# weikaolun/horovod-distributed-example

Hardware: AMD Instinct MI355X
Metric: images/sec (whole node) + scaling efficiency, ResNet-50 bf16 at 1/2/4/8 MI355X (higher is better)
Workload: dtype bf16; 1 GPU; model=ResNet-50, global_batch=2048, per_gpu_batch=2048, image=224, parallelism=dp1, optimizer=mivod FusedSGD via DistributedOptimizer, compression=none, transport=local, hip_graph=False

## Files before the change

csrc/kernels/mv_stem.hip:

```cpp
#include "mv_mfma.h"
#include "mv_stem.h"

namespace mv {
namespace stem {

constexpr int kH = 224, kW = 224, kC = 4, kOH = 112, kOW = 112, kCO = 64;
constexpr int kPW = 232;
constexpr int kChunks = 32;
#ifndef MV_STEM_ROWS
#define MV_STEM_ROWS 2
#endif
constexpr int kR = MV_STEM_ROWS;
constexpr int kIR = 2 * kR + 5;
constexpr int kPatch = kIR * kPW;
constexpr int kLoads = (kIR * 230 + 255) / 256;

__device__ __forceinline__ u32x2 ld_px(const __bf16* x, int64_t pix, int cin) {
  if (cin == 4) return *reinterpret_cast<const u32x2*>(x + pix * 4);
  const uint16_t* p = reinterpret_cast<const uint16_t*>(x) + pix * 3;
  return u32x2{(uint32_t)p[0] | ((uint32_t)p[1] << 16), (uint32_t)p[2]};
}

__global__ __launch_bounds__(256, 2) void stem_fwd_kernel(const __bf16* __restrict__ x,
                                                       const __bf16* __restrict__ w,
                                                       __bf16* __restrict__ z,
                                                       const float* __restrict__ shift,
                                                       float* __restrict__ partial, int N,
                                                       int cin) {
  __shared__ __attribute__((aligned(16))) __bf16 ws[kCO * kChunks * 8];
  __shared__ __attribute__((aligned(16))) __bf16 ps[kPatch * kC];
  const int tid = threadIdx.x, lane = tid & 63, wv = tid >> 6;
  const int g = lane >> 4, rl = lane & 15;

  for (int q = tid; q < kCO * kChunks; q += 256) {
    const int o = q / kChunks, ch = q % kChunks;
    u32x4 v = {0u, 0u, 0u, 0u};
    if (ch < 28) {
      const int r = ch / 4, pr = ch % 4;
      const __bf16* src = w + ((o * 7 + r) * 7 + 2 * pr) * kC;
      const u32x2 a = *reinterpret_cast<const u32x2*>(src);
      v[0] = a[0];
      v[1] = a[1];
      if (pr < 3) {
        const u32x2 b = *reinterpret_cast<const u32x2*>(src + kC);
        v[2] = b[0];
        v[3] = b[1];
      }
    }
    *reinterpret_cast<u32x4*>(ws + (o * kChunks + (ch ^ (o & 7))) * 8) = v;
  }

  const int64_t rows = (int64_t)N * (kOH / kR);
  u32x2 pre[kLoads];
  auto gload = [&](int64_t row) {
    const int n = (int)(row / (kOH / kR)), oh = (int)(row % (kOH / kR)) * kR;
#pragma unroll
    for (int i = 0; i < kLoads; ++i) {
      const int q = tid + i * 256;
      const int r = q / 230, pc = q % 230;
      const int ih = 2 * oh + r - 3, iw = pc - 3;
      u32x2 v = {0u, 0u};
      if (q < kIR * 230 && ih >= 0 && ih < kH && iw >= 0 && iw < kW)
        v = ld_px(x, ((int64_t)n * kH + ih) * kW + iw, cin);
      pre[i] = v;
    }
  };

  float sh[4], s1[4], s2[4];
#pragma unroll
  for (int j = 0; j < 4; ++j) {
    sh[j] = shift ? shift[16 * wv + 4 * g + j] : 0.f;
    s1[j] = 0.f;
    s2[j] = 0.f;
  }
  int64_t row = blockIdx.x;
  if (row < rows) gload(row);
  for (; row < rows; row += gridDim.x) {
    __syncthreads();
#pragma unroll
    for (int i = 0; i < kLoads; ++i) {
      const int q = tid + i * 256;
      if (q < kIR * 230) {
        const int r = q / 230, pc = q % 230;
        *reinterpret_cast<u32x2*>(ps + (r * kPW + pc) * kC) = pre[i];
      }
    }
    __syncthreads();
    if (row + gridDim.x < rows) gload(row + gridDim.x);
    f32x4v acc[kR][7];
#pragma unroll
    for (int j = 0; j < kR; ++j)
#pragma unroll
      for (int t = 0; t < 7; ++t) acc[j][t] = f32x4v{0.f, 0.f, 0.f, 0.f};
#pragma unroll
    for (int kk = 0; kk < 7; ++kk) {
      const int o = 16 * wv + rl, ch = kk * 4 + g;
      const bf16x8 wf = *reinterpret_cast<const bf16x8*>(ws + (o * kChunks + (ch ^ (o & 7))) * 8);
#pragma unroll
      for (int j = 0; j < kR; ++j)
#pragma unroll
        for (int t = 0; t < 7; ++t) {
          const int p = t * 16 + rl;
          const bf16x8 af = *reinterpret_cast<const bf16x8*>(
              ps + ((2 * j + kk) * kPW + 2 * p + 2 * g) * kC);
          acc[j][t] = mfma(wf, af, acc[j][t]);
        }
    }
#pragma unroll
    for (int j = 0; j < kR; ++j)
#pragma unroll
    for (int t = 0; t < 7; ++t) {
      __bf16* zr = z + (row * kR + j) * (int64_t)kOW * kCO + 16 * wv + 4 * g;
      const int p = t * 16 + rl;
      const uint32_t lo = cvt_pk_bf16_cc(acc[j][t][0], acc[j][t][1]);
      const uint32_t hi = cvt_pk_bf16_cc(acc[j][t][2], acc[j][t][3]);
      *reinterpret_cast<u32x2*>(zr + (int64_t)p * kCO) = u32x2{lo, hi};
      const float v[4] = {__uint_as_float(lo << 16), __uint_as_float(lo & 0xffff0000u),
                          __uint_as_float(hi << 16), __uint_as_float(hi & 0xffff0000u)};
#pragma unroll
      for (int e = 0; e < 4; ++e) {
        const float d = v[e] - sh[e];
        s1[e] += d;
        s2[e] += d * d;
      }
    }
  }
#pragma unroll
  for (int j = 0; j < 4; ++j) {
#pragma unroll
    for (int o = 1; o < 16; o <<= 1) {
      s1[j] += __shfl_xor(s1[j], o, kWave);
      s2[j] += __shfl_xor(s2[j], o, kWave);
    }
  }
  if (rl == 0) {
#pragma unroll
    for (int j = 0; j < 4; ++j) {
      const int c = 16 * wv + 4 * g + j;
      partial[((int64_t)blockIdx.x * 2 + 0) * kCO + c] = s1[j];
      partial[((int64_t)blockIdx.x * 2 + 1) * kCO + c] = s2[j];
    }
  }
}

}
}

int mv_stem_partials(int N) {
  static int per = [] {
    int v = 0;
    if (hipOccupancyMaxActiveBlocksPerMultiprocessor(&v, (const void*)mv::stem::stem_fwd_kernel,
                                                     256, 0) != hipSuccess || v < 1)
      v = 1;
    return v;
  }();
  const int64_t rows = (int64_t)N * (mv::stem::kOH / mv::stem::kR);
  int64_t g = (int64_t)mv::num_cus() * per;
  if (g > rows) g = rows;
  return (int)g;
}

void mv_stem_fwd(const void* x, const void* w, void* z, const float* shift, float* partial, int N,
                 hipStream_t st, int grid, int cin) {
  if (grid <= 0) grid = mv_stem_partials(N);
  hipLaunchKernelGGL(mv::stem::stem_fwd_kernel, dim3(grid), dim3(256), 0, st, (const __bf16*)x,
                     (const __bf16*)w, (__bf16*)z, shift, partial, N, cin);
}

namespace mv {
namespace stem {


__device__ __forceinline__ s16x4 px_tr4(const __bf16* ps, int p0, int r, int s0, int c) {
  int p = p0 + (c >> 2);
  p = p < kOW - 1 ? p : kOW - 1;
  const __bf16* a = ps + (r * kPW + 2 * p + s0) * kC + 4 * (c & 3);
  return lds_tr4(a);
}

constexpr int kPairs = (kOW / 2) * 8;

__device__ __forceinline__ void pool_bn_dz_pair(const MvStemPoolBwd& pb, const float* coef, int n,
                                                int oh, int b, int c, const u32x4 (&zr)[2],
                                                u32x4 (&out)[2]) {
  constexpr int kPH = kOH / 2, kPW2 = kOW / 2;
  float acc[2][8];
#pragma unroll
  for (int k = 0; k < 2; ++k)
#pragma unroll
    for (int e = 0; e < 8; ++e) acc[k][e] = 0.f;
  const int a = oh >> 1, i = oh & 1;
  const int nda = i && a + 1 < kPH ? 2 : 1;
  const bool ok1 = b + 1 < kPW2;
  for (int da = 0; da < nda; ++da) {
    const int kh = i - 2 * da + 1;
    u32x2 iw[2];
    u32x4 dv[2], d2v[2];
#pragma unroll
    for (int db = 0; db < 2; ++db) {
      const int col = db && !ok1 ? b : b + db;
      const int64_t o = (((int64_t)n * kPH + a + da) * kPW2 + col) * kCO + c;
      iw[db] = *reinterpret_cast<const u32x2*>(pb.idx + o);
      dv[db] = *reinterpret_cast<const u32x4*>(reinterpret_cast<const __bf16*>(pb.dy) + o);
      d2v[db] = pb.dy2 ? *reinterpret_cast<const u32x4*>(reinterpret_cast<const __bf16*>(pb.dy2) + o)
                       : u32x4{0u, 0u, 0u, 0u};
    }
#pragma unroll
    for (int db = 0; db < 2; ++db) {
      float d[8];
#pragma unroll
      for (int q = 0; q < 4; ++q) {
        d[2 * q] = __uint_as_float(dv[db][q] << 16);
        d[2 * q + 1] = __uint_as_float(dv[db][q] & 0xffff0000u);
      }
      if (pb.dy2) {
#pragma unroll
        for (int q = 0; q < 4; ++q) {
          d[2 * q] += __uint_as_float(d2v[db][q] << 16);
          d[2 * q + 1] += __uint_as_float(d2v[db][q] & 0xffff0000u);
        }
      }
#pragma unroll
      for (int jj = 0; jj < 2; ++jj) {
        const int kw = jj - 2 * db + 1;
        if (kw < 0) continue;
        const uint32_t pos = db && !ok1 ? 0xffu : (uint32_t)(kh * 3 + kw);
#pragma unroll
        for (int e = 0; e < 8; ++e) {
          const uint32_t wd = e < 4 ? iw[db][0] : iw[db][1];
          if (((wd >> (8 * (e & 3))) & 0xffu) == pos) acc[jj][e] += d[e];
        }
      }
    }
  }
#pragma unroll
  for (int k = 0; k < 2; ++k) {
    float v[8];
#pragma unroll
    for (int q = 0; q < 4; ++q) {
      v[2 * q] = __uint_as_float(zr[k][q] << 16);
      v[2 * q + 1] = __uint_as_float(zr[k][q] & 0xffff0000u);
    }
#pragma unroll
    for (int e = 0; e < 8; ++e) {
      const float* kf = coef + c + e;
      const float d = __builtin_fmaf(v[e], kf[0], kf[64]) > 0.f ? acc[k][e] : 0.f;
      v[e] = __builtin_fmaf(kf[128], d, __builtin_fmaf(kf[192], v[e], kf[256]));
    }
    out[k] = u32x4{cvt_pk_bf16(v[0], v[1]), cvt_pk_bf16(v[2], v[3]), cvt_pk_bf16(v[4], v[5]),
                   cvt_pk_bf16(v[6], v[7])};
  }
}

template <int NT, bool FUSE>
__global__ __launch_bounds__(NT, FUSE ? 4 : 1) void stem_wgrad_kernel(const __bf16* __restrict__ x,
                                                        const __bf16* __restrict__ dz,
                                                        float* __restrict__ partial, int N,
                                                        int cin, MvStemPoolBwd pb) {
  static_assert(!FUSE || NT >= kPairs, "one pixel pair per thread");
  constexpr int kTPW = 14 / (NT / 256);
  __shared__ __attribute__((aligned(16))) __bf16 ps[7 * kPW * kC];
  __shared__ __attribute__((aligned(16))) __bf16 ds[128 * 64];
  __shared__ float coef[FUSE ? 5 * 64 : 1];
  const int tid = threadIdx.x;
  if constexpr (FUSE) {
    for (int q = tid; q < 5 * 64; q += NT) {
      const float* src[5] = {pb.scale, pb.bias, pb.ca, pb.cb, pb.cc};
      coef[q] = src[q / 64][q % 64];
    }
  }
  const int64_t rows = (int64_t)N * kOH;
  f32x4v acc[kTPW];
#pragma unroll
  for (int t = 0; t < kTPW; ++t) acc[t] = f32x4v{0.f, 0.f, 0.f, 0.f};
  for (int q = tid; q < 16 * 8; q += NT) {
    const int r = 112 + q / 8, ch = q % 8;
    *reinterpret_cast<u32x4*>(ds + r * 64 + ((ch ^ tr_swz4(r)) << 3)) = u32x4{0u, 0u, 0u, 0u};
  }
  constexpr int kPL = (7 * 230 + NT - 1) / NT;
  constexpr int kDz = FUSE ? 2 : (kOW * 8 + NT - 1) / NT;
  u32x2 pp[kPL];
  u32x4 pd[kDz];
  auto gload = [&](int64_t row, int tid) {
    const int n = (int)(row / kOH), oh = (int)(row % kOH);
#pragma unroll
    for (int i = 0; i < kPL; ++i) {
      const int q = tid + i * NT;
      const int r = q / 230, pc = q % 230;
      const int ih = 2 * oh + r - 3, iw = pc - 3;
      u32x2 v = {0u, 0u};
      if (q < 7 * 230 && ih >= 0 && ih < kH && iw >= 0 && iw < kW)
        v = ld_px(x, ((int64_t)n * kH + ih) * kW + iw, cin);
      pp[i] = v;
    }
    if constexpr (FUSE) {
      const __bf16* zr = reinterpret_cast<const __bf16*>(pb.z) + row * (int64_t)kOW * kCO;
      const int b = tid / 8, c = (tid % 8) * 8;
#pragma unroll
      for (int k = 0; k < 2; ++k)
        pd[k] = tid < kPairs ? *reinterpret_cast<const u32x4*>(zr + (2 * b + k) * kCO + c)
                             : u32x4{0u, 0u, 0u, 0u};

    } else {
      const __bf16* dzr = dz + row * (int64_t)kOW * kCO;
#pragma unroll
      for (int i = 0; i < kDz; ++i) {
        const int q = tid + i * NT;
        pd[i] = q < kOW * 8 ? *reinterpret_cast<const u32x4*>(dzr + q * 8) : u32x4{0u, 0u, 0u, 0u};
      }
    }
  };
  int64_t row = blockIdx.x;
  if (row < rows) gload(row, tid);
  for (; row < rows; row += gridDim.x) {
    int tid = threadIdx.x;
    if constexpr (FUSE) asm volatile("" : "+v"(tid));
    const int lane = tid & 63, wv = tid >> 6, g = lane >> 4, cl = lane & 15;
    const int cw = wv & 3, t0 = (wv >> 2) * kTPW;
    __syncthreads();
#pragma unroll
    for (int i = 0; i < kPL; ++i) {
      const int q = tid + i * NT;
      if (q < 7 * 230) {
        const int r = q / 230, pc = q % 230;
        *reinterpret_cast<u32x2*>(ps + (r * kPW + pc) * kC) = pp[i];
      }
    }
    if constexpr (FUSE) {
      if (tid < kPairs) {
        const int oh = (int)(row % kOH);
        const int b = tid / 8, ch = tid % 8;
        const u32x4 zr[2] = {pd[0], pd[1]};
        u32x4 o[2];
        pool_bn_dz_pair(pb, coef, (int)(row / kOH), oh, b, ch * 8, zr, o);
#pragma unroll
        for (int k = 0; k < 2; ++k) {
          const int r = 2 * b + k;
          *reinterpret_cast<u32x4*>(ds + r * 64 + ((ch ^ tr_swz4(r)) << 3)) = o[k];
        }
      }
    } else {
#pragma unroll
      for (int i = 0; i < kDz; ++i) {
        const int q = tid + i * NT;
        if (q < kOW * 8) {
          const int r = q / 8, ch = q % 8;
          *reinterpret_cast<u32x4*>(ds + r * 64 + ((ch ^ tr_swz4(r)) << 3)) = pd[i];
        }
      }
    }
    __syncthreads();
    if (row + gridDim.x < rows) gload(row + gridDim.x, tid);
#pragma unroll
    for (int ks = 0; ks < 4; ++ks) {
      const int p0 = ks * 32 + 8 * g;
      const bf16x8 af = cat8_copy(tr4_swz4<false>(ds, p0, 16 * cw, cl),
                                  tr4_swz4<false>(ds, p0 + 4, 16 * cw, cl));
#pragma unroll
      for (int tt = 0; tt < kTPW; ++tt) {
        const int t = t0 + tt, r = t >> 1, s0 = 4 * (t & 1);
        const bf16x8 bf = cat8_copy(px_tr4(ps, p0, r, s0, cl), px_tr4(ps, p0 + 4, r, s0, cl));
        acc[tt] = mfma(af, bf, acc[tt]);
      }
      if constexpr (FUSE) __builtin_amdgcn_sched_barrier(0);
    }
  }
  const int lane = tid & 63, wv = tid >> 6, g = lane >> 4, cl = lane & 15;
  const int cw = wv & 3, t0 = (wv >> 2) * kTPW;
  float* pout = partial + (int64_t)blockIdx.x * kCO * 224;
#pragma unroll
  for (int tt = 0; tt < kTPW; ++tt)
#pragma unroll
    for (int r = 0; r < 4; ++r)
      pout[(16 * cw + 4 * g + r) * 224 + (t0 + tt) * 16 + cl] = acc[tt][r];
}

__global__ __launch_bounds__(256) void stem_wgrad_reduce_kernel(const float* __restrict__ partial,
                                                                int G, __bf16* __restrict__ dw) {
  const int i = blockIdx.x * 256 + threadIdx.x;
  if (i >= kCO * 7 * 7 * kC) return;
  const int c = i % kC, s = (i / kC) % 7, r = (i / (kC * 7)) % 7, o = i / (kC * 49);
  const int k = r * 32 + s * 4 + c;
  float a0 = 0.f, a1 = 0.f, a2 = 0.f, a3 = 0.f;
  int gi = 0;
  for (; gi + 3 < G; gi += 4) {
    a0 += partial[((int64_t)gi * kCO + o) * 224 + k];
    a1 += partial[((int64_t)(gi + 1) * kCO + o) * 224 + k];
    a2 += partial[((int64_t)(gi + 2) * kCO + o) * 224 + k];
    a3 += partial[((int64_t)(gi + 3) * kCO + o) * 224 + k];
  }
  for (; gi < G; ++gi) a0 += partial[((int64_t)gi * kCO + o) * 224 + k];
  dw[i] = (__bf16)((a0 + a1) + (a2 + a3));
}

}
}

int mv_stem_wgrad_blocks(int N) {
  int64_t g = (int64_t)mv::num_cus() * 4;
  const int64_t rows = (int64_t)N * mv::stem::kOH;
  if (g > rows) g = rows;
  return (int)g;
}

void mv_stem_wgrad(const void* x, const void* dz, void* dw, float* work, int N, hipStream_t st,
                   int cin) {
  const int G = mv_stem_wgrad_blocks(N);
  hipLaunchKernelGGL((mv::stem::stem_wgrad_kernel<256, false>), dim3(G), dim3(256), 0, st,
                     (const __bf16*)x, (const __bf16*)dz, work, N, cin, MvStemPoolBwd{});
  hipLaunchKernelGGL(mv::stem::stem_wgrad_reduce_kernel, dim3((64 * 196 + 255) / 256), dim3(256), 0,
                     st, work, G, (__bf16*)dw);
}

void mv_stem_wgrad_pool_bn(const void* x, const MvStemPoolBwd& pb, void* dw, float* work, int N,
                           hipStream_t st, int cin) {
  const int G = mv_stem_wgrad_blocks(N);
  hipLaunchKernelGGL((mv::stem::stem_wgrad_kernel<512, true>), dim3(G), dim3(512), 0, st,
                     (const __bf16*)x, (const __bf16*)nullptr, work, N, cin, pb);
  hipLaunchKernelGGL(mv::stem::stem_wgrad_reduce_kernel, dim3((64 * 196 + 255) / 256), dim3(256), 0,
                     st, work, G, (__bf16*)dw);
}
```

Baseline: 18840 images/sec.

## Use contiguous row ranges with sliding-window LDS ring for stem fwd/wgrad input reuse

Switches the stem forward and weight-gradient kernels from a strided row schedule to contiguous per-block row ranges. Input patch rows are kept in a duplicated LDS ring buffer, so each step only loads the new stride rows instead of the full 7x7 window. In the fused wgrad path, maxpool gradient, index and dy2 rows are prefetched into LDS with async global-to-LDS loads and double-buffered, instead of being read directly from global memory per pixel pair. This cuts redundant global loads but adds LDS footprint, extra ring stores, wait_vm synchronisation and full reloads at image boundaries, which can lower occupancy.

```diff
diff --git a/csrc/kernels/mv_stem.hip b/csrc/kernels/mv_stem.hip
--- a/csrc/kernels/mv_stem.hip
+++ b/csrc/kernels/mv_stem.hip
@@ -12,8 +12,11 @@
 #endif
 constexpr int kR = MV_STEM_ROWS;
 constexpr int kIR = 2 * kR + 5;
-constexpr int kPatch = kIR * kPW;
-constexpr int kLoads = (kIR * 230 + 255) / 256;
+constexpr int kNew = 2 * kR;
+constexpr int kRingF = 2 * kIR - 1;
+constexpr int kPatch = kRingF * kPW;
+constexpr int kLoads = (kNew * 230 + 255) / 256;
+constexpr int kFull = (kIR * 230 + 255) / 256;
 
 __device__ __forceinline__ u32x2 ld_px(const __bf16* x, int64_t pix, int cin) {
   if (cin == 4) return *reinterpret_cast<const u32x2*>(x + pix * 4);
@@ -51,16 +54,23 @@
   }
 
   const int64_t rows = (int64_t)N * (kOH / kR);
+  const int64_t row0 = (int64_t)blockIdx.x * rows / gridDim.x;
+  const int64_t row1 = ((int64_t)blockIdx.x + 1) * rows / gridDim.x;
   u32x2 pre[kLoads];
+  auto ring_store = [&](int q , int pc, u32x2 v) {
+    const int pos = q % kIR;
+    *reinterpret_cast<u32x2*>(ps + (pos * kPW + pc) * kC) = v;
+    if (pos < kIR - 1) *reinterpret_cast<u32x2*>(ps + ((pos + kIR) * kPW + pc) * kC) = v;
+  };
   auto gload = [&](int64_t row) {
     const int n = (int)(row / (kOH / kR)), oh = (int)(row % (kOH / kR)) * kR;
 #pragma unroll
     for (int i = 0; i < kLoads; ++i) {
       const int q = tid + i * 256;
       const int r = q / 230, pc = q % 230;
-      const int ih = 2 * oh + r - 3, iw = pc - 3;
+      const int ih = 2 * oh + kIR - kNew - 3 + r, iw = pc - 3;
       u32x2 v = {0u, 0u};
-      if (q < kIR * 230 && ih >= 0 && ih < kH && iw >= 0 && iw < kW)
+      if (q < kNew * 230 && ih < kH && iw >= 0 && iw < kW)
         v = ld_px(x, ((int64_t)n * kH + ih) * kW + iw, cin);
       pre[i] = v;
     }
@@ -73,20 +83,36 @@
     s1[j] = 0.f;
     s2[j] = 0.f;
   }
-  int64_t row = blockIdx.x;
-  if (row < rows) gload(row);
-  for (; row < rows; row += gridDim.x) {
+  for (int64_t row = row0; row < row1; ++row) {
+    const int n = (int)(row / (kOH / kR)), oh = (int)(row % (kOH / kR)) * kR;
     __syncthreads();
-#pragma unroll
-    for (int i = 0; i < kLoads; ++i) {
-      const int q = tid + i * 256;
-      if (q < kIR * 230) {
+    if (row == row0 || oh == 0) {
+      u32x2 fl[kFull];
+#pragma unroll
+      for (int i = 0; i < kFull; ++i) {
+        const int q = tid + i * 256;
         const int r = q / 230, pc = q % 230;
-        *reinterpret_cast<u32x2*>(ps + (r * kPW + pc) * kC) = pre[i];
+        const int ih = 2 * oh + r - 3, iw = pc - 3;
+        u32x2 v = {0u, 0u};
+        if (q < kIR * 230 && ih >= 0 && ih < kH && iw >= 0 && iw < kW)
+          v = ld_px(x, ((int64_t)n * kH + ih) * kW + iw, cin);
+        fl[i] = v;
+      }
+#pragma unroll
+      for (int i = 0; i < kFull; ++i) {
+        const int q = tid + i * 256;
+        if (q < kIR * 230) ring_store(2 * oh + q / 230, q % 230, fl[i]);
+      }
+    } else {
+#pragma unroll
+      for (int i = 0; i < kLoads; ++i) {
+        const int q = tid + i * 256;
+        if (q < kNew * 230) ring_store(2 * oh + kIR - kNew + q / 230, q % 230, pre[i]);
       }
     }
     __syncthreads();
-    if (row + gridDim.x < rows) gload(row + gridDim.x);
+    if (row + 1 < row1) gload(row + 1);
+    const __bf16* pw = ps + ((2 * oh) % kIR) * (kPW * kC);
     f32x4v acc[kR][7];
 #pragma unroll
     for (int j = 0; j < kR; ++j)
@@ -102,7 +128,7 @@
         for (int t = 0; t < 7; ++t) {
           const int p = t * 16 + rl;
           const bf16x8 af = *reinterpret_cast<const bf16x8*>(
-              ps + ((2 * j + kk) * kPW + 2 * p + 2 * g) * kC);
+              pw + ((2 * j + kk) * kPW + 2 * p + 2 * g) * kC);
           acc[j][t] = mfma(wf, af, acc[j][t]);
         }
     }
@@ -180,7 +206,33 @@
 
 constexpr int kPairs = (kOW / 2) * 8;
 
-__device__ __forceinline__ void pool_bn_dz_pair(const MvStemPoolBwd& pb, const float* coef, int n,
+constexpr int kPoolRow = (kOW / 2) * kCO;
+constexpr int kSlotDy2 = kPoolRow * 2, kSlotIdx = kPoolRow * 4;
+constexpr int kSlot = kSlotIdx + 4096;
+
+template <int NT>
+__device__ __forceinline__ void pool_row_issue(const MvStemPoolBwd& pb, unsigned char* pl, int n,
+                                               int a, int wv, int lane) {
+  const int64_t o = ((int64_t)n * (kOH / 2) + a) * kPoolRow;
+  unsigned char* s = pl + (a & 1) * kSlot;
+  const int nld = pb.dy2 ? 18 : 11;
+  for (int j = wv; j < nld; j += NT / 64) {
+    const int jj = !pb.dy2 && j >= 7 ? j + 7 : j;
+    if (jj < 7) {
+      glds16(reinterpret_cast<const unsigned char*>(pb.dy) + o * 2 + jj * 1024 + lane * 16,
+             reinterpret_cast<__bf16*>(s + jj * 1024));
+    } else if (jj < 14) {
+      glds16(reinterpret_cast<const unsigned char*>(pb.dy2) + o * 2 + (jj - 7) * 1024 + lane * 16,
+             reinterpret_cast<__bf16*>(s + kSlotDy2 + (jj - 7) * 1024));
+    } else {
+      int b = (jj - 14) * 1024 + lane * 16;
+      b = b < kPoolRow ? b : 0;
+      glds16(pb.idx + o + b, reinterpret_cast<__bf16*>(s + kSlotIdx + (jj - 14) * 1024));
+    }
+  }
+}
+
+__device__ __forceinline__ void pool_bn_dz_pair(const unsigned char* pl, bool has2, const float* coef,
                                                 int oh, int b, int c, const u32x4 (&zr)[2],
                                                 u32x4 (&out)[2]) {
   constexpr int kPH = kOH / 2, kPW2 = kOW / 2;
@@ -194,16 +246,16 @@
   const bool ok1 = b + 1 < kPW2;
   for (int da = 0; da < nda; ++da) {
     const int kh = i - 2 * da + 1;
+    const unsigned char* s = pl + ((a + da) & 1) * kSlot;
     u32x2 iw[2];
     u32x4 dv[2], d2v[2];
 #pragma unroll
     for (int db = 0; db < 2; ++db) {
       const int col = db && !ok1 ? b : b + db;
-      const int64_t o = (((int64_t)n * kPH + a + da) * kPW2 + col) * kCO + c;
-      iw[db] = *reinterpret_cast<const u32x2*>(pb.idx + o);
-      dv[db] = *reinterpret_cast<const u32x4*>(reinterpret_cast<const __bf16*>(pb.dy) + o);
-      d2v[db] = pb.dy2 ? *reinterpret_cast<const u32x4*>(reinterpret_cast<const __bf16*>(pb.dy2) + o)
-                       : u32x4{0u, 0u, 0u, 0u};
+      const int o = col * kCO + c;
+      iw[db] = *reinterpret_cast<const u32x2*>(s + kSlotIdx + o);
+      dv[db] = *reinterpret_cast<const u32x4*>(s + o * 2);
+      d2v[db] = has2 ? *reinterpret_cast<const u32x4*>(s + kSlotDy2 + o * 2) : u32x4{0u, 0u, 0u, 0u};
     }
 #pragma unroll
     for (int db = 0; db < 2; ++db) {
@@ -213,7 +265,7 @@
         d[2 * q] = __uint_as_float(dv[db][q] << 16);
         d[2 * q + 1] = __uint_as_float(dv[db][q] & 0xffff0000u);
       }
-      if (pb.dy2) {
+      if (has2) {
 #pragma unroll
         for (int q = 0; q < 4; ++q) {
           d[2 * q] += __uint_as_float(d2v[db][q] << 16);
@@ -251,6 +303,8 @@
                    cvt_pk_bf16(v[6], v[7])};
   }
 }
+
+constexpr int kRing = 13;
 
 template <int NT, bool FUSE>
 __global__ __launch_bounds__(NT, FUSE ? 4 : 1) void stem_wgrad_kernel(const __bf16* __restrict__ x,
@@ -259,8 +313,9 @@
                                                         int cin, MvStemPoolBwd pb) {
   static_assert(!FUSE || NT >= kPairs, "one pixel pair per thread");
   constexpr int kTPW = 14 / (NT / 256);
-  __shared__ __attribute__((aligned(16))) __bf16 ps[7 * kPW * kC];
+  __shared__ __attribute__((aligned(16))) __bf16 ps[kRing * kPW * kC];
   __shared__ __attribute__((aligned(16))) __bf16 ds[128 * 64];
+  __shared__ __attribute__((aligned(16))) unsigned char pl[FUSE ? 2 * kSlot : 16];
   __shared__ float coef[FUSE ? 5 * 64 : 1];
   const int tid = threadIdx.x;
   if constexpr (FUSE) {
@@ -270,6 +325,8 @@
     }
   }
   const int64_t rows = (int64_t)N * kOH;
+  const int64_t row0 = (int64_t)blockIdx.x * rows / gridDim.x;
+  const int64_t row1 = ((int64_t)blockIdx.x + 1) * rows / gridDim.x;
   f32x4v acc[kTPW];
 #pragma unroll
   for (int t = 0; t < kTPW; ++t) acc[t] = f32x4v{0.f, 0.f, 0.f, 0.f};
@@ -277,19 +334,24 @@
     const int r = 112 + q / 8, ch = q % 8;
     *reinterpret_cast<u32x4*>(ds + r * 64 + ((ch ^ tr_swz4(r)) << 3)) = u32x4{0u, 0u, 0u, 0u};
   }
-  constexpr int kPL = (7 * 230 + NT - 1) / NT;
+  constexpr int kPL = (2 * 230 + NT - 1) / NT;
   constexpr int kDz = FUSE ? 2 : (kOW * 8 + NT - 1) / NT;
   u32x2 pp[kPL];
   u32x4 pd[kDz];
+  auto ring_store = [&](int q , int pc, u32x2 v) {
+    const int pos = q % 7;
+    *reinterpret_cast<u32x2*>(ps + (pos * kPW + pc) * kC) = v;
+    if (pos < kRing - 7) *reinterpret_cast<u32x2*>(ps + ((pos + 7) * kPW + pc) * kC) = v;
+  };
   auto gload = [&](int64_t row, int tid) {
     const int n = (int)(row / kOH), oh = (int)(row % kOH);
 #pragma unroll
     for (int i = 0; i < kPL; ++i) {
       const int q = tid + i * NT;
       const int r = q / 230, pc = q % 230;
-      const int ih = 2 * oh + r - 3, iw = pc - 3;
+      const int ih = 2 * oh + 2 + r, iw = pc - 3;
       u32x2 v = {0u, 0u};
-      if (q < 7 * 230 && ih >= 0 && ih < kH && iw >= 0 && iw < kW)
+      if (q < 2 * 230 && ih < kH && iw >= 0 && iw < kW)
         v = ld_px(x, ((int64_t)n * kH + ih) * kW + iw, cin);
       pp[i] = v;
     }
@@ -310,29 +372,46 @@
       }
     }
   };
-  int64_t row = blockIdx.x;
-  if (row < rows) gload(row, tid);
-  for (; row < rows; row += gridDim.x) {
+  if (row0 < row1) gload(row0, tid);
+  for (int64_t row = row0; row < row1; ++row) {
     int tid = threadIdx.x;
     if constexpr (FUSE) asm volatile("" : "+v"(tid));
     const int lane = tid & 63, wv = tid >> 6, g = lane >> 4, cl = lane & 15;
     const int cw = wv & 3, t0 = (wv >> 2) * kTPW;
+    const int n = (int)(row / kOH), oh = (int)(row % kOH);
+    const bool full = row == row0 || oh == 0;
+    if constexpr (FUSE) wait_vm<0>();
     __syncthreads();
-#pragma unroll
-    for (int i = 0; i < kPL; ++i) {
-      const int q = tid + i * NT;
-      if (q < 7 * 230) {
+    if (full) {
+#pragma unroll 1
+      for (int q = tid; q < 7 * 230; q += NT) {
         const int r = q / 230, pc = q % 230;
-        *reinterpret_cast<u32x2*>(ps + (r * kPW + pc) * kC) = pp[i];
+        const int ih = 2 * oh + r - 3, iw = pc - 3;
+        u32x2 v = {0u, 0u};
+        if (ih >= 0 && ih < kH && iw >= 0 && iw < kW)
+          v = ld_px(x, ((int64_t)n * kH + ih) * kW + iw, cin);
+        ring_store(2 * oh + r, pc, v);
+      }
+      if constexpr (FUSE) {
+        const int wu = __builtin_amdgcn_readfirstlane(wv);
+        pool_row_issue<NT>(pb, pl, n, oh >> 1, wu, lane);
+        if ((oh >> 1) + 1 < kOH / 2) pool_row_issue<NT>(pb, pl, n, (oh >> 1) + 1, wu, lane);
+        wait_vm<0>();
+        __syncthreads();
+      }
+    } else {
+#pragma unroll
+      for (int i = 0; i < kPL; ++i) {
+        const int q = tid + i * NT;
+        if (q < 2 * 230) ring_store(2 * oh + 5 + q / 230, q % 230, pp[i]);
       }
     }
     if constexpr (FUSE) {
       if (tid < kPairs) {
-        const int oh = (int)(row % kOH);
         const int b = tid / 8, ch = tid % 8;
         const u32x4 zr[2] = {pd[0], pd[1]};
         u32x4 o[2];
-        pool_bn_dz_pair(pb, coef, (int)(row / kOH), oh, b, ch * 8, zr, o);
+        pool_bn_dz_pair(pl, pb.dy2 != nullptr, coef, oh, b, ch * 8, zr, o);
 #pragma unroll
         for (int k = 0; k < 2; ++k) {
           const int r = 2 * b + k;
@@ -350,7 +429,8 @@
       }
     }
     __syncthreads();
-    if (row + gridDim.x < rows) gload(row + gridDim.x, tid);
+    if (row + 1 < row1) gload(row + 1, tid);
+    const __bf16* pw = ps + ((2 * oh) % 7) * (kPW * kC);
 #pragma unroll
     for (int ks = 0; ks < 4; ++ks) {
       const int p0 = ks * 32 + 8 * g;
@@ -359,10 +439,15 @@
 #pragma unroll
       for (int tt = 0; tt < kTPW; ++tt) {
         const int t = t0 + tt, r = t >> 1, s0 = 4 * (t & 1);
-        const bf16x8 bf = cat8_copy(px_tr4(ps, p0, r, s0, cl), px_tr4(ps, p0 + 4, r, s0, cl));
+        const bf16x8 bf = cat8_copy(px_tr4(pw, p0, r, s0, cl), px_tr4(pw, p0 + 4, r, s0, cl));
         acc[tt] = mfma(af, bf, acc[tt]);
       }
       if constexpr (FUSE) __builtin_amdgcn_sched_barrier(0);
+    }
+    if constexpr (FUSE) {
+      const int a = oh >> 1;
+      if ((oh & 1) && a + 2 < kOH / 2 && row + 2 < row1)
+        pool_row_issue<NT>(pb, pl, n, a + 2, __builtin_amdgcn_readfirstlane(wv), lane);
     }
   }
   const int lane = tid & 63, wv = tid >> 6, g = lane >> 4, cl = lane & 15;
```

New measurement: 18980 images/sec, median of 6. About the same (+0.8%).
